# WxuanYuan/diffusynth

Measured on AMD Instinct MI355X. Metric: denoising-steps/sec (batch x T) on 256x64 latents, higher is better.
Workload: dtype bf16x3; 1 GPU; BASELINE configs[2]: DiffSynthSampler.sample() wall-clock, production ConditionedUnet (random init, torch.manual_seed(0)), bf16x3 (fp32 tensors, dense convolutions as 3 bf16 MFMA terms with fp32 accumulation: meets 1e-3 vs the fp32 reference), batch 64/GPU, latent (4,256,64), text condition, CFG=6.0 (U-Net batch 128 per step), 33-step respaced ddpm schedule, Philox noise on device; global_batch=64, parallelism=batch-shard x1, weights replicated

## Files before the change

### __graft_entry__.py

```python
import glob
import os
import subprocess
import sys

ROOT = os.path.dirname(os.path.abspath(__file__))
CSRC = os.path.join(ROOT, "diffusynth_amd", "csrc")
LIB = os.path.join(ROOT, "diffusynth_amd", "libdiffusynth_hip.so")
HIPCC = os.environ.get("HIPCC", "/opt/rocm/bin/hipcc")


NOSLP = {"conv3x3_halo3.hip", "conv3x3_halo3_hp.hip", "conv_quad_halo3.hip", "conv_quad_halo3_split.hip", "conv3x3_smalln.hip", "conv_igemm.hip", "conv_splitk.hip", "conv1x1_x3.hip", "attn_fused.hip", "attn_x3.hip", "dec_final.hip", "conv3x3_c80.hip", "convt4x4_c80.hip"}


def _compile(src, obj, flags):
    extra = ["-fno-slp-vectorize"] if (os.path.basename(src) in NOSLP and os.environ.get("DS_BUILD_SLP") != "1") else []
    cmd = [HIPCC, "--offload-arch=gfx950", "-O3", "-std=c++17", "-fPIC", "-c", "-o", obj, src] + extra + flags
    print("[build]", " ".join(cmd), flush=True)
    subprocess.check_call(cmd)


def build_lib(lib=LIB, flags=(), objdir=None, force=False):
    from concurrent.futures import ThreadPoolExecutor
    srcs = sorted(glob.glob(os.path.join(CSRC, "*.hip")))
    hdrs = glob.glob(os.path.join(CSRC, "*.hpp")) + [os.path.join(ROOT, "include", "diffusynth_hip.h")]
    objdir = objdir or os.path.join(ROOT, "build", os.path.splitext(os.path.basename(lib))[0])
    os.makedirs(objdir, exist_ok=True)
    stamp = os.path.join(objdir, "flags.txt")
    want = " ".join(sorted(flags)) + " | noslp: " + " ".join(sorted(NOSLP)) + " | slp=" + os.environ.get("DS_BUILD_SLP", "0") + " | " + HIPCC
    have = open(stamp).read() if os.path.exists(stamp) else None
    if have != want:
        force = True
        if os.path.exists(stamp):
            os.remove(stamp)
    newest_hdr = max(os.path.getmtime(h) for h in hdrs)
    jobs, objs = [], []
    for s in srcs:
        o = os.path.join(objdir, os.path.basename(s)[:-4] + ".o")
        objs.append(o)
        if force or not os.path.exists(o) or os.path.getmtime(o) < max(os.path.getmtime(s), newest_hdr):
            jobs.append((s, o))
    if jobs:
        with ThreadPoolExecutor(max_workers=min(len(jobs), os.cpu_count() or 4)) as ex:
            list(ex.map(lambda so: _compile(so[0], so[1], list(flags)), jobs))
    if jobs or not os.path.exists(lib) or os.path.getmtime(lib) < max(os.path.getmtime(o) for o in objs):
        cmd = [HIPCC, "--offload-arch=gfx950", "-fPIC", "-shared", "-o", lib] + objs
        print("[build]", " ".join(cmd), flush=True)
        subprocess.check_call(cmd)
    with open(stamp, "w") as f:
        f.write(want)
    return lib


BOUNDS_LIB = os.path.join(ROOT, "diffusynth_amd", "libdiffusynth_hip_bounds.so")


def build_bounds(force=False):
    return build_lib(BOUNDS_LIB, flags=["-DDS_BOUNDS=1"], force=force)


def build(force=False):
    build_lib(force=force)
    if os.environ.get("DS_BUILD_BOUNDS", "1") != "0":
        try:
            build_bounds(force=force)
# ... 62 lines not shown
```

### diffusynth_amd/csrc/conv3x3_halo3.hip

```cpp
#include "conv3x3_halo3_kernel.hpp"

int ds_conv3x3_halo3_hp_run(const ds_conv_params* p, dim3 grid, bool pair, hipStream_t st);

int ds_conv3x3_halo3_parts(const ds_conv_params* p) {
    const int twl = halo_twl(p->W), TW = 1 << twl, TH = BM >> twl;
    return ((p->H + TH - 1) / TH) * ((p->W + TW - 1) / TW) * (p->cout_pad / BN);
}

static int halo3_batch(const ds_conv_params* p) { return p->batch_hint > 0 ? p->batch_hint : p->B; }

int ds_conv3x3_halo3_launch(const ds_conv_params* p, hipStream_t st) {
    DS_REQUIRE(p->dtype == DS_BF16, "conv3x3_halo3: bf16 only");
    DS_REQUIRE(p->KH == 3 && p->KW == 3 && p->stride == 1 && p->pad_h == 1 && p->pad_w == 1 && !p->transposed,
               "conv3x3_halo3: 3x3 stride 1 pad 1 only");
    DS_REQUIRE(p->C1 == 0 && p->C0 % 32 == 0, "conv3x3_halo3: single source, Cin multiple of 32 (got %d+%d)", p->C0, p->C1);
    DS_REQUIRE(p->Ho == p->H && p->Wo == p->W && !p->out_nchw_f32, "conv3x3_halo3: same-size NHWC output only");
    DS_REQUIRE(p->cout_pad % BN == 0 && p->wk_order == 1, "conv3x3_halo3: cout_pad %% 96 == 0 and chunk-major weights (wk_order = 1)");
    const bool split_in = (p->flags & DS_CONV_F_SPLIT_IN) != 0;
    DS_REQUIRE(p->ksplit <= 1 || (p->slab && (p->flags == 0 || split_in) && ((split_in ? p->C0 / 64 : p->C0 / 32) % p->ksplit) == 0 && !p->res_steps),
               "conv3x3_halo3: ksplit=%d needs a slab, must divide the %d source chunks and excludes the fused res_conv", p->ksplit, split_in ? p->C0 / 64 : p->C0 / 32);
    const int out_mode = (p->flags >> 1) & 3;
    DS_REQUIRE(out_mode <= 2 && (p->flags & ~7) == 0, "conv3x3_halo3: unknown flags %d", p->flags);
    DS_REQUIRE(!split_in || (p->C0 % 64 == 0 && !p->res_steps), "conv3x3_halo3: split input needs C0 = 2C with C %% 32 == 0 and no fused res_conv");
    DS_REQUIRE(p->flags == 0 || split_in, "conv3x3_halo3: the split-precision launches (flags != 0) take a split input (DS_CONV_F_SPLIT_IN)");
    DS_REQUIRE(out_mode == 0 || !p->res_steps, "conv3x3_halo3: split / fp32 output excludes the fused res_conv");
    DS_REQUIRE(out_mode != 2 || p->act == DS_ACT_NONE, "conv3x3_halo3: fp32 output has no activation variant");
    DS_REQUIRE(!p->res || out_mode == 2 || p->flags == 0, "conv3x3_halo3: in the split-precision modes a residual needs the fp32 output");
    DS_REQUIRE(out_mode != 1 || p->out_C >= p->out_c0 + 2 * p->Cout, "conv3x3_halo3: split output needs out_C >= 2 Cout");
    const int nchunks = split_in ? (p->C0 / 32) * 3 / 2 : p->C0 / 32;
    if (p->res_steps) {
        DS_REQUIRE(!p->res, "conv3x3_halo3: a fused res_conv excludes a residual tensor");
        DS_REQUIRE(p->res_src0 && p->res_C0 > 0 && p->res_C0 % 32 == 0 && p->res_C1 % 32 == 0 && p->res_steps == (p->res_C0 + p->res_C1) / 32 &&
                       p->res_steps % 3 == 0,
                   "conv3x3_halo3: res_conv channels (%d,%d) must be multiples of 32 (96 in total) and res_steps = their chunks", p->res_C0, p->res_C1);
        DS_REQUIRE(p->res_C1 == 0 || (p->res_src1 && p->res_H1 > 0 && p->res_W1 > 0), "conv3x3_halo3: second res_conv source incomplete");
        DS_REQUIRE(ds_aligned16(p->res_src0) && (!p->res_C1 || ds_aligned16(p->res_src1)), "conv3x3_halo3: res_conv sources must be 16-byte aligned");
    }
    DS_REQUIRE((long long)p->H * p->W * (p->C0 > p->res_C0 ? p->C0 : p->res_C0) * 2 < (1ll << 31) &&
                   (long long)(nchunks * 9 + p->res_steps) * p->cout_pad * 64 < (1ll << 31),
               "conv3x3_halo3: one sample / the packed weights must stay below 2 GiB (32-bit buffer offsets)");
    DS_REQUIRE((long long)p->H * p->W * p->out_C * (out_mode == 2 ? 4 : 2) < (1ll << 31), "conv3x3_halo3: one output sample must stay below 2 GiB (32-bit buffer offsets)");
    const int twl = halo_twl(p->W), TW = 1 << twl, TH = BM >> twl;
    const bool pair = p->flags != 0 && twl == 3 && 2 * p->H <= TH && p->W <= TW && p->ksplit <= 1 && !p->res_steps && halo3_batch(p) >= 2;
    dim3 grid(((p->H + TH - 1) / TH) * ((p->W + TW - 1) / TW), p->cout_pad / BN, pair ? (p->B + 1) / 2 : p->B * (p->ksplit > 1 ? p->ksplit : 1));
    {
        static DsDevOnce once;
        int dev;
        if (once.need(&dev)) {
            float h[GELU_TAB_N];
            auto T = [](double a) { return a * 0.5 * erfc(a * 0.70710678118654752440); };
            for (int i = 0; i < GELU_TAB_N; ++i) {
                const unsigned lo = (unsigned)(GELU_TAB_BASE + i) << 16, hi = lo + 0x10000u;
                float flo, fhi;
                memcpy(&flo, &lo, 4);
                memcpy(&fhi, &hi, 4);
                h[i] = (float)T(0.5 * ((double)flo + (double)fhi));
            }
            hipError_t e = hipMemcpyToSymbol(HIP_SYMBOL(g_gelu_lut), h, sizeof(h));
            if (e != hipSuccess) DS_FAIL(DS_ELAUNCH, "conv3x3_halo3: GELU table upload: %s", hipGetErrorString(e));
            once.done(dev);
        }
    }
    return p->flags ? ds_conv3x3_halo3_hp_run(p, grid, pair, st) : halo3_run<false>(*p, grid, false, st);
}

#if DS_BOUNDS
extern "C" int ds_bounds_fetch_conv_halo3(ds_bounds_rec* out, int reset) { return ds_bounds_fetch_tu(out, reset); }
#endif
```

### diffusynth_amd/csrc/conv3x3_halo3_kernel.hpp

```cpp
#pragma once
#include "common.hpp"
#ifndef DS_STAMP
#define DS_STAMP 0
#endif
#if DS_BOUNDS
void ds_conv_bounds_table(const ds_conv_params& p, int kernel, int stats_parts, ds_bx* out);
#endif

#include "conv_halo3_common.hpp"

namespace {

__device__ __attribute__((aligned(16))) float g_gelu_lut[GELU_TAB_N];

constexpr int hp_tile(int s) { return s < 18 ? (s & 1) * 9 + (s >> 1) : s; }
constexpr int hp_tile_ahead(int s, int d) { return s + d < 27 ? hp_tile(s + d) : 27 + hp_tile(s + d - 27); }
template <int FIRST, int... I, class F>
__device__ __forceinline__ void hp_steps(std::integer_sequence<int, I...>, F&& f) { (f(std::integral_constant<int, FIRST + I>{}), ...); }

#ifdef DS_FORCE_VGPRS
#define DS_VGPR_ATTR __attribute__((amdgpu_num_vgpr(DS_FORCE_VGPRS)))
#else
#define DS_VGPR_ATTR
#endif
template <int TWL, bool HP, bool PAIR = false>
__global__ __launch_bounds__(NT, PAIR ? 1 : DS_MINBLK) DS_VGPR_ATTR void conv3x3_halo3_kernel(const ds_conv_params p) {
    static_assert(!PAIR || (HP && TWL == 3), "two samples per block: the 8 x 32 tile of the split-precision instantiation");
    using G = HG<TWL>;
    constexpr int TW = G::TW, TH = G::TH, HCP = G::HCP, NPX = G::NPX, H_IT = G::H_IT, HH0 = G::HH0, HH1 = G::HH1;
    extern __shared__ __attribute__((aligned(16))) char smem[];
    float* const shl = reinterpret_cast<float*>(smem + OFF_SHL);
    float* const red = reinterpret_cast<float*>(smem + OFF_B);

    const int tid = threadIdx.x, lane = tid & 63, wave = tid >> 6;
    const long st_k0 = DS_STAMP ? __builtin_amdgcn_s_memrealtime() : 0;
    const int m = lane & 15, q = lane >> 4;
    const int tiles_w = (p.W + TW - 1) >> TWL;
    const int gx = gridDim.x, gy = gridDim.y, nwg = gx * gy * gridDim.z;
    int wid = blockIdx.x + gx * (blockIdx.y + gy * blockIdx.z);
    if ((nwg & 7) == 0) wid = (wid & 7) * (nwg >> 3) + (wid >> 3);
    constexpr int NGROUP = 2;
    int by, bxz;
    if (gy % NGROUP == 0 && gy > NGROUP) {
        const int lo = wid % NGROUP, t = wid / NGROUP, nxz = gx * (int)gridDim.z;
        bxz = t % nxz;
        by = (t / nxz) * NGROUP + lo;
    } else {
        by = wid % gy;
        bxz = wid / gy;
    }
    const int bx = bxz % gx, bz = bxz / gx;
    const int th = bx / tiles_w, tw = bx - th * tiles_w;
    const int h0 = th * TH, w0 = tw * TW;
    const int ksplit = p.ksplit > 1 ? p.ksplit : 1;
    const int b = (PAIR ? 2 : 1) * (bz / ksplit), kz = bz - (bz / ksplit) * ksplit, n0 = by * BN;
    const bool has2 = PAIR && b + 1 < p.B;
    constexpr bool split_in = HP;
    const int Cin = p.C0, NSRC = Cin >> 5;
    const int NCC = (split_in ? NSRC + (NSRC >> 1) : NSRC) / ksplit;
    const int cc_lo = kz * NCC;
    const int nsteps = NCC * 9;
    auto src_chunk = [&](int cc) {
        const int v = cc_lo + cc;
        if (!split_in) return v;
        const int c = v / 3, j = v - 3 * c;
        return j == 2 ? (NSRC >> 1) + c : c;
    };

    const int NR = (HP || ksplit > 1) ? 0 : p.res_steps, R0 = p.res_C0 >> 5;
    const char* const wbase = reinterpret_cast<const char*>(p.wpk);
    const unsigned wbytes = (unsigned)(NCC * ksplit * 9 + p.res_steps) * p.cout_pad * 64;
    const rsrc_t rs_w = __builtin_amdgcn_make_buffer_rsrc(const_cast<char*>(wbase), (short)0, (int)wbytes, 0x00020000);

    unsigned hvo[H_IT];
    rsrc_t rs_h;
    const char* hbase;
    int h_buf = DS_BX_SRC0;
    auto use_source = [&](const void* ptr, int sH, int sW, int sC, int offh, int offw, bool centre_only, int bounds_buf) {
        hbase = reinterpret_cast<const char*>(ptr) + (size_t)b * sH * sW * sC * 2;
        rs_h = __builtin_amdgcn_make_buffer_rsrc(const_cast<char*>(hbase), (short)0, (int)((unsigned)sH * sW * sC * 2) * (has2 ? 2 : 1), 0x00020000);
// ... 47 lines not shown
    };
    auto store_b = [&](auto slotc, auto bufc) {
        constexpr int sl = decltype(slotc)::value, buf = decltype(bufc)::value;
        *reinterpret_cast<u32x4*>(smem + buf * B_STRIDE + bst0) = rb[sl][0];
        *reinterpret_cast<u32x4*>(smem + buf * B_STRIDE + bst1) = rb[sl][1];
    };
    auto load_halo_to = [&](u32x4* dst, auto halfc) {
        constexpr int half = decltype(halfc)::value, n = half ? HH1 : HH0;
#pragma unroll
        for (int k = 0; k < n; ++k) dst[k] = buf_ld16(rs_h, hbase, hvo[half * HH0 + k], h_so, h_buf);
    };
    auto load_halo = [&](auto halfc) { load_halo_to(rh, halfc); };
    auto store_halo_from = [&](const u32x4* src, auto bufc, auto halfc) {
        constexpr int buf = decltype(bufc)::value, half = decltype(halfc)::value, n = half ? HH1 : HH0;
#pragma unroll
        for (int k = 0; k < n; ++k) *reinterpret_cast<u32x4*>(smem + lds_h + buf * G::HB + (half * HH0 + k) * 64 * PSTR) = src[k];
    };
    auto store_halo = [&](auto bufc, auto halfc) { store_halo_from(rh, bufc, halfc); };

    int xb[XT];
#pragma unroll
    for (int i = 0; i < XT; ++i) {
        int row_l, col_l;
        halo_tile_rc<TWL>(wave, i, m, row_l, col_l);
        const int hp0 = (row_l + (PAIR ? 2 * (row_l >> 4) : 0)) * HCP + col_l;
        xb[i] = OFF_H + hp0 * PSTR + ((q ^ (((hp0 >> 2) & 1) << 1)) << 4);
    }
    static_assert(((HCP >> 2) & 1) == 1 && ((2 * HCP >> 2) & 1) == 0, "tap-row swizzle flips assume HCP / 4 odd");
    const int xm1 = ((m & 3) == 3) << 5, xm2 = ((m & 3) >= 2) << 5;
    const int xm1n = xm1 ^ 32, xm2n = xm2 ^ 32;
    const int bw = OFF_B + W_ROW0(m) * PSTR + ((q ^ ((-(m >> 2)) & 3)) << 4);

    bf16x8 fx[2][XT], fw[WT];
    auto read_x = [&](auto setc, auto tyc, auto txc, int imm) {
        constexpr int set = decltype(setc)::value, ty = decltype(tyc)::value, tx = decltype(txc)::value;
#pragma unroll
        for (int i = 0; i < XT; ++i) {
            int a = xb[i];
            if constexpr (HP) {
                if constexpr (tx == 1) a ^= xm1;
                if constexpr (tx == 2) a ^= xm2;
                if constexpr (ty == 1) {
                    if constexpr (tx != 0) asm volatile("" : "+v"(a));
                    a ^= 32;
                }
            } else {
                if constexpr (tx == 0 && ty == 1) a ^= 32;
                if constexpr (tx == 1) a ^= (ty == 1 ? xm1n : xm1);
                if constexpr (tx == 2) a ^= (ty == 1 ? xm2n : xm2);
            }
            fx[set][i] = *reinterpret_cast<const bf16x8*>(smem + a + (ty * HCP + tx) * PSTR + imm);
        }
    };
#ifndef DS_HALO3_ABL
#define DS_HALO3_ABL 0
#endif
    auto read_w = [&](int j, int imm) { fw[j] = *reinterpret_cast<const bf16x8*>(smem + bw + EPI_CH(j) * PSTR + imm); };
    f32x4 acc[XT][WT];
    auto mma_j = [&](auto setc, int j) {
        constexpr int set = decltype(setc)::value;
#pragma unroll
        for (int i = 0; i < XT; ++i) acc[i][j] = __builtin_amdgcn_mfma_f32_16x16x32_bf16(fw[j], fx[set][i], acc[i][j], 0, 0, 0);
    };
    using I0 = std::integral_constant<int, 0>;
    using I1 = std::integral_constant<int, 1>;
    using I2 = std::integral_constant<int, 2>;

    GnPartialLoads gnl;
    const bool raw = ksplit > 1;
    if (p.gn_part && !raw) gn_partials_issue(p.gn_part, p.gn_parts, b, gnl);
    const bool fold = !raw && CONV_FOLD(p);
    const int ncls = fold ? p.ncls : 1;
    constexpr int ST_IT = (10 * BN + NT - 1) / NT;
#if !DS_BOUNDS
    float t1v[ST_IT], t2v[ST_IT], rbv[ST_IT];
    {
        auto tab = [&](const float* ptr, int n) {
            return __builtin_amdgcn_make_buffer_rsrc(const_cast<char*>(ptr ? reinterpret_cast<const char*>(ptr) : wbase), (short)0, ptr ? n * 4 : 0, 0x00020000);
        };
        const bool use_bias = !fold && p.bias && !raw;
        const rsrc_t rs_t1 = tab(fold ? p.fold_t1 : (use_bias ? p.bias : nullptr), fold ? ncls * p.Cout : p.Cout);
        const rsrc_t rs_t2 = tab(fold ? p.fold_t2 : nullptr, ncls * p.Cout);
        const rsrc_t rs_rb = tab((NR > 0 && p.res_bias) ? p.res_bias : nullptr, p.Cout);
#pragma unroll
        for (int k = 0; k < ST_IT; ++k) {
            const int e = tid + k * NT, cls = e / BN, n = n0 + e - cls * BN;
            const unsigned bad = ((unsigned)(e >= ncls * BN) | (unsigned)(n >= p.Cout)) << 31;
            const unsigned o = (unsigned)((fold ? cls * p.Cout : 0) + n) * 4u;
            t1v[k] = __builtin_bit_cast(float, __builtin_amdgcn_raw_buffer_load_b32(rs_t1, (int)((o & 0x7fffffffu) | bad), 0, 0));
            t2v[k] = __builtin_bit_cast(float, __builtin_amdgcn_raw_buffer_load_b32(rs_t2, (int)((o & 0x7fffffffu) | bad), 0, 0));
            rbv[k] = NR > 0 ? __builtin_bit_cast(float, __builtin_amdgcn_raw_buffer_load_b32(rs_rb, (int)((((unsigned)n * 4u) & 0x7fffffffu) | bad), 0, 0)) : 0.f;
        }
    }
#endif
    const bool use_lut = !HP && G::LUT && p.act == DS_ACT_GELU && !raw;
    static_assert(GELU_TAB_N * 4 <= 2 * NT * 16 && GELU_TAB_N % 4 == 0, "the table is staged as two 16-byte vectors per thread");
    u32x4 lutv = {0u, 0u, 0u, 0u}, lutv2 = {0u, 0u, 0u, 0u};
    if (use_lut) {
        lutv = *reinterpret_cast<const u32x4*>(reinterpret_cast<const char*>(g_gelu_lut) + tid * 16);
        lutv2 = *reinterpret_cast<const u32x4*>(reinterpret_cast<const char*>(g_gelu_lut) + (NT + min(tid, GELU_TAB_N / 4 - NT - 1)) * 16);
    }
    const long st_p1 = DS_STAMP ? __builtin_amdgcn_s_memrealtime() : 0;
    u32x4 rh2[HH0];
    h_so = NR > 0 ? 0u : (unsigned)src_chunk(0) * 64u;
    load_halo_to(rh2, I0{});
    load_halo(I1{});
    if constexpr (HP) {
        load_b_at(I0{}, hp_tile(0));
        load_b_at(I1{}, hp_tile(1));
    } else {
        load_b(I0{});
        load_b(I1{});
    }
    float gn_a = 1.f, gn_am = 0.f;
    if (raw) {
    } else if (p.gn_part) gn_partials_finish(gnl, p.gn_part, p.gn_parts, p.gn_count, p.gn_eps, b, gn_a, gn_am);
    else if (p.gn_ab) {
        gn_a = DS_LD(float, p.gn_ab + 2 * b, DS_BX_GNAB);
        gn_am = DS_LD(float, p.gn_ab + 2 * b + 1, DS_BX_GNAB);
    }
    if constexpr (PAIR) {
        const int b1 = has2 ? b + 1 : b;
        float a1 = 1.f, am1 = 0.f;
        if (p.gn_part) gn_from_partials(p.gn_part, p.gn_parts, p.gn_count, p.gn_eps, b1, a1, am1);
        else if (p.gn_ab) {
            a1 = DS_LD(float, p.gn_ab + 2 * b1, DS_BX_GNAB);
            am1 = DS_LD(float, p.gn_ab + 2 * b1 + 1, DS_BX_GNAB);
        }
        if (tid == 0) {
            reinterpret_cast<float*>(smem + G::LDS)[0] = a1;
            reinterpret_cast<float*>(smem + G::LDS)[1] = am1;
        }
    }
#if DS_BOUNDS
    conv_shift_table<BN, 10, NT>(raw ? conv_kslice_view(p) : p, fold, n0, gn_am, NR > 0 ? p.res_bias : nullptr, shl);
#else
#pragma unroll
    for (int k = 0; k < ST_IT; ++k) {
        const int e = tid + k * NT;
        if (e < 10 * BN) shl[e] = (t1v[k] + rbv[k]) - gn_am * t2v[k];
    }
#endif
    const long st_p2 = DS_STAMP ? __builtin_amdgcn_s_memrealtime() : 0;
#pragma unroll
    for (int i = 0; i < XT; ++i)
#pragma unroll
        for (int j = 0; j < WT; ++j) acc[i][j] = f32x4{0.f, 0.f, 0.f, 0.f};
    if (use_lut) {
        *reinterpret_cast<u32x4*>(smem + G::OFF_LUT + tid * 16) = lutv;
        if (tid < GELU_TAB_N / 4 - NT) *reinterpret_cast<u32x4*>(smem + G::OFF_LUT + (NT + tid) * 16) = lutv2;
    }
    store_halo_from(rh2, I0{}, I0{});
    store_halo(I0{}, I1{});
    store_b(I0{}, I0{});
    store_b(I1{}, I1{});
    if constexpr (HP) {
        load_b_at(I2{}, hp_tile(2));
        load_b_at(I0{}, hp_tile(3));
        load_b_at(I1{}, hp_tile(4));
    } else {
        load_b(I2{});
        load_b(I0{});
        load_b(I1{});
    }
    __syncthreads();

    if constexpr (!HP) if (NR > 0) {
        set_res_src(1);
        load_halo_to(rh, I0{});
        load_halo_to(rh + HH0, I1{});
        auto res_step = [&](auto hbc, auto phc, int r) {
            constexpr int hb = decltype(hbc)::value, ph = decltype(phc)::value, rs = (ph + 2) % 3;
            read_x(I0{}, I1{}, I1{}, hb * G::HB);
#pragma unroll
            for (int j = 0; j < WT; ++j) read_w(j, ph * B_STRIDE);
            __builtin_amdgcn_sched_barrier(0);
            store_halo_from(rh, std::integral_constant<int, hb ^ 1>{}, I0{});
            store_halo_from(rh + HH0, std::integral_constant<int, hb ^ 1>{}, I1{});
            store_b(std::integral_constant<int, rs>{}, std::integral_constant<int, rs>{});
            __builtin_amdgcn_sched_barrier(0);
            load_b(std::integral_constant<int, rs>{});
            if (r + 2 <= NR) {
                set_res_src(r + 2);
                __builtin_amdgcn_sched_barrier(0);
                load_halo_to(rh, I0{});
                load_halo_to(rh + HH0, I1{});
            }
            __builtin_amdgcn_sched_barrier(0);
#pragma unroll
            for (int j = 0; j < WT; ++j) mma_j(I0{}, j);
            __builtin_amdgcn_sched_barrier(0);
            __syncthreads();
        };
        for (int r = 0; r < NR; r += 6) {
            res_step(I0{}, I0{}, r);
            res_step(I1{}, I1{}, r + 1);
            res_step(I0{}, I2{}, r + 2);
            if (r + 3 < NR) {
                res_step(I1{}, I0{}, r + 3);
                res_step(I0{}, I1{}, r + 4);
                res_step(I1{}, I2{}, r + 5);
            }
        }
        const float inv_a = 1.0f / gn_a;
#pragma unroll
        for (int i = 0; i < XT; ++i)
#pragma unroll
            for (int j = 0; j < WT; ++j)
#pragma unroll
                for (int r = 0; r < 4; ++r) acc[i][j][r] *= inv_a;
    }
    const int par = HP ? 0 : (NR & 1);
    if (par) read_x(I1{}, I0{}, I0{}, G::HB);
    else read_x(I0{}, I0{}, I0{}, 0);
#pragma unroll
    for (int j = 0; j < WT; ++j) read_w(j, 0);

    auto chunk = [&](auto hbufc, int cc) {
        constexpr int hbuf = decltype(hbufc)::value;
        h_so = (unsigned)src_chunk(cc + 1 < NCC ? cc + 1 : cc) * 64u;
        auto step = [&](auto tapc) {
            constexpr int tap = decltype(tapc)::value;
            constexpr int rs = (tap + 2) % 3;
            constexpr int cur = (tap + hbuf) & 1;
            constexpr int ntap = (tap + 1) % 9, nty = ntap / 3, ntx = ntap % 3, nhb = tap == 8 ? (hbuf ^ 1) : hbuf;
            constexpr int nW = 2 + (tap == 3 ? HH0 : (tap == 7 ? HH1 : 0)), nV = 2 + (tap == 1 ? HH0 : (tap == 4 ? HH1 : 0));
            if constexpr (tap == 3) store_halo(std::integral_constant<int, hbuf ^ 1>{}, I0{});
            if constexpr (tap == 7) store_halo(std::integral_constant<int, hbuf ^ 1>{}, I1{});
            store_b(std::integral_constant<int, rs>{}, std::integral_constant<int, rs>{});
            load_b(std::integral_constant<int, rs>{});
            if constexpr (tap == 1) load_halo(I0{});
            if constexpr (tap == 4) load_halo(I1{});
            mma_j(std::integral_constant<int, (DS_HALO3_ABL & 2) ? 0 : cur>{}, 0);
            if constexpr (!(DS_HALO3_ABL & 1)) read_w(0, ((tap + 1) % 3) * B_STRIDE);
            if constexpr (!(DS_HALO3_ABL & 2))
                read_x(std::integral_constant<int, cur ^ 1>{}, std::integral_constant<int, nty>{}, std::integral_constant<int, ntx>{}, nhb * G::HB);
#pragma unroll
            for (int j = 1; j < WT; ++j) {
                mma_j(std::integral_constant<int, (DS_HALO3_ABL & 2) ? 0 : cur>{}, j);
                if constexpr (!(DS_HALO3_ABL & 1)) read_w(j, ((tap + 1) % 3) * B_STRIDE);
            }
#pragma unroll
            for (int k = 0; k < nW; ++k) { SGB(SG_MFMA, 1); SGB(SG_DSW, 1); }
#pragma unroll
            for (int k = 0; k < nV; ++k) { SGB(SG_MFMA, 1); SGB(SG_VMEM, 1); }
            constexpr int L0 = nW + nV;
#pragma unroll
            for (int k = 0; k < 5; ++k) { SGB(SG_MFMA, 1); SGB(SG_DSR, 1); }
            constexpr int L1 = L0 + 5;
#pragma unroll
            for (int j = 1; j < WT; ++j) {
                const int before = (4 * j + 4 > L1 + j - 1 ? 4 * j + 4 : L1 + j - 1);
                const int prev = j == 1 ? L1 : (4 * (j - 1) + 4 > L1 + j - 2 ? 4 * (j - 1) + 4 : L1 + j - 2);
                if (before - prev == 1) SGB(SG_MFMA, 1);
                else if (before - prev == 2) SGB(SG_MFMA, 2);
                else if (before - prev == 3) SGB(SG_MFMA, 3);
                else if (before - prev == 4) SGB(SG_MFMA, 4);
                else if (before - prev == 5) SGB(SG_MFMA, 5);
                else if (before - prev == 6) SGB(SG_MFMA, 6);
                else if (before - prev == 7) SGB(SG_MFMA, 7);
                SGB(SG_DSR, 1);
            }
            __builtin_amdgcn_sched_barrier(0);
#if DS_BOUNDS || defined(DS_LGKM0)
            asm volatile("s_waitcnt lgkmcnt(0)" ::: "memory");
#else
// ... 17 lines not shown
        constexpr bool pairs = s < 18, rx = !pairs || (s & 1);
        constexpr int tap = pairs ? s >> 1 : s - 18;
        constexpr int rs = (s + 2) % 3;
        constexpr int cur = (tap + (pairs ? 0 : 1)) & 1;
        constexpr int ntap = (tap + 1) % 9, nty = ntap / 3, ntx = ntap % 3, nhb = (pairs ? 0 : 1) ^ (tap == 8 ? 1 : 0);
        constexpr int ld0 = pairs ? 2 : 19, st0 = pairs ? 6 : 21, ld1 = pairs ? 8 : 22, st1 = pairs ? 14 : 25;
        constexpr int nW = 2 + (s == st0 ? HH0 : (s == st1 ? HH1 : 0)), nV = 2 + (s == ld0 ? HH0 : (s == ld1 ? HH1 : 0));
        constexpr int NX = (rx && !(DS_HALO3_ABL & 2)) ? XT : 0;
        if constexpr (s == st0) store_halo(std::integral_constant<int, pairs ? 1 : 0>{}, I0{});
        if constexpr (s == st1) store_halo(std::integral_constant<int, pairs ? 1 : 0>{}, I1{});
        store_b(std::integral_constant<int, rs>{}, std::integral_constant<int, rs>{});
        load_b_at(std::integral_constant<int, rs>{}, hp_tile_ahead(s, 5));
        if constexpr (s == ld0) load_halo(I0{});
        if constexpr (s == ld1) load_halo(I1{});
        mma_j(std::integral_constant<int, (DS_HALO3_ABL & 2) ? 0 : cur>{}, 0);
        if constexpr (!(DS_HALO3_ABL & 1)) read_w(0, ((s + 1) % 3) * B_STRIDE);
        if constexpr (NX > 0)
            read_x(std::integral_constant<int, cur ^ 1>{}, std::integral_constant<int, nty>{}, std::integral_constant<int, ntx>{}, nhb * G::HB);
#pragma unroll
        for (int j = 1; j < WT; ++j) {
            mma_j(std::integral_constant<int, (DS_HALO3_ABL & 2) ? 0 : cur>{}, j);
            if constexpr (!(DS_HALO3_ABL & 1)) read_w(j, ((s + 1) % 3) * B_STRIDE);
        }
#pragma unroll
        for (int k = 0; k < nW; ++k) { SGB(SG_MFMA, 1); SGB(SG_DSW, 1); }
#pragma unroll
        for (int k = 0; k < nV; ++k) { SGB(SG_MFMA, 1); SGB(SG_VMEM, 1); }
#pragma unroll
        for (int k = 0; k < 1 + NX; ++k) { SGB(SG_MFMA, 1); SGB(SG_DSR, 1); }
        constexpr int L1 = nW + nV + 1 + NX;
#pragma unroll
        for (int j = 1; j < WT; ++j) {
            const int before = (4 * j + 4 > L1 + j - 1 ? 4 * j + 4 : L1 + j - 1);
            const int prev = j == 1 ? L1 : (4 * (j - 1) + 4 > L1 + j - 2 ? 4 * (j - 1) + 4 : L1 + j - 2);
            if (before - prev == 1) SGB(SG_MFMA, 1);
            else if (before - prev == 2) SGB(SG_MFMA, 2);
            else if (before - prev == 3) SGB(SG_MFMA, 3);
            else if (before - prev == 4) SGB(SG_MFMA, 4);
            else if (before - prev == 5) SGB(SG_MFMA, 5);
            else if (before - prev == 6) SGB(SG_MFMA, 6);
            else if (before - prev == 7) SGB(SG_MFMA, 7);
            SGB(SG_DSR, 1);
        }
        __builtin_amdgcn_sched_barrier(0);
#if DS_BOUNDS || defined(DS_LGKM0)
        asm volatile("s_waitcnt lgkmcnt(0)" ::: "memory");
#else
        if constexpr (rx) asm volatile("s_waitcnt lgkmcnt(10)" ::: "memory");
        else asm volatile("s_waitcnt lgkmcnt(6)" ::: "memory");
#endif
        if constexpr (!(DS_HALO3_ABL & 4)) __builtin_amdgcn_s_barrier();
        __builtin_amdgcn_sched_barrier(0);
    };
    long st_t0 = 0, st_r0 = 0;
    if constexpr (DS_STAMP) {
        st_t0 = __builtin_amdgcn_s_memtime();
        st_r0 = __builtin_amdgcn_s_memrealtime();
        __builtin_amdgcn_s_waitcnt(0xC07F);
    }
    if constexpr (HP) {
        for (int cc = 0; cc < NCC; cc += 3) {
            h_so = (unsigned)src_chunk(cc + 2) * 64u;
            hp_steps<0>(std::make_integer_sequence<int, 18>{}, hp_step);
            h_so = (unsigned)src_chunk(cc + 3 < NCC ? cc + 3 : cc) * 64u;
            hp_steps<18>(std::make_integer_sequence<int, 9>{}, hp_step);
            w_c += 27u * wstep;
        }
    } else {
        int cc0 = 0;
        if (par) {
            chunk(I1{}, 0);
            cc0 = 1;
        }
        for (int cc = cc0; cc < NCC; cc += 2) {
            chunk(I0{}, cc);
            if (cc + 1 < NCC) chunk(I1{}, cc + 1);
        }
    }

#pragma unroll
    for (int i = 0; i < XT; ++i) {
        asm volatile("" ::"v"(fx[0][i]));
        asm volatile("" ::"v"(fx[1][i]));
    }
#pragma unroll
    for (int j = 0; j < WT; ++j) asm volatile("" ::"v"(fw[j]));
    if constexpr (DS_STAMP) {
        const long st_t1 = __builtin_amdgcn_s_memtime();
        if (p.slab && lane == 0) {
            long* d = reinterpret_cast<long*>(p.slab) + ((size_t)(bz * gy + by) * gx + bx) * 32 + wave * 8;
            d[0] = st_t1 - st_t0; d[1] = st_p1 - st_k0; d[2] = st_p2 - st_k0; d[3] = nsteps;
            d[4] = st_r0 - st_k0; d[5] = __builtin_amdgcn_s_memrealtime() - st_r0; d[6] = st_k0;
        }
    }
    auto at = [&](int row_l, int col_l) {
        ConvCoord c;
        if constexpr (PAIR) {
            const int smp = row_l >> 4;
            c.ho = row_l & 15;
            c.wo = w0 + col_l;
            c.ok = c.ho < p.H && c.wo < p.W && (!smp || has2);
            c.pix = (smp * p.H + c.ho) * p.W + c.wo;
            return c;
        }
        c.ho = h0 + row_l;
        c.wo = w0 + col_l;
        c.ok = c.ho < p.H && c.wo < p.W;
        c.pix = c.ho * p.W + c.wo;
        return c;
    };
    auto coord2 = [&](int i, int mm) { int row_l, col_l; halo_tile_rc<TWL>(wave, i, mm, row_l, col_l); return at(row_l, col_l); };
    auto coord = [&](int i) { return coord2(i, m); };
    char* const stage = smem + OFF_H + wave * EPI_F32_WAVE;
    static_assert(4 * EPI_F32_WAVE <= 2 * G::HB, "the staging tiles fit the halo buffers");
    float s1 = 0.f, s2 = 0.f;
    const int outHW = p.H * p.W;
    const long st_e1 = DS_STAMP ? __builtin_amdgcn_s_memrealtime() : 0;
    const int out_mode = HP ? (p.flags >> 1) & 3 : 0;
    const float* shl_w = shl;
    float ga_w = gn_a;
    int b_e = b, outHW_e = outHW;
    if constexpr (PAIR) {
        const float gn_a1 = reinterpret_cast<const float*>(smem + G::LDS)[0], gn_am1 = reinterpret_cast<const float*>(smem + G::LDS)[1];
        float* const shl1 = reinterpret_cast<float*>(smem + OFF_H + 4 * EPI_F32_WAVE);
        static_assert(4 * EPI_F32_WAVE + SHL_BYTES <= 2 * G::HB, "the second shift table fits the halo buffers too");
        conv_shift_table<BN, 10, NT>(p, fold, n0, gn_am1, nullptr, shl1);
        __syncthreads();
        if (__builtin_amdgcn_readfirstlane(wave) >= 2) {
            shl_w = shl1;
            ga_w = gn_a1;
        }
        b_e = b >> 1;
        outHW_e = 2 * outHW;
    }
    if (raw) {
        halo3_epilogue_hp<DS_ACT_NONE, 2>(conv_kslice_view(p), acc, kz * p.B + b, n0, outHW, shl, coord, s1, s2, 1.0f, lane);
// ... 6 lines not shown
        else halo3_epilogue_rows_f32<true, false>(p, acc, b_e, n0, outHW_e, shl_w, coord, coord2, stage, s1, s2, ga_w, lane);
      } else {
        if (p.act == DS_ACT_GELU) halo3_epilogue<DS_ACT_GELU, true, false>(p, acc, b_e, n0, outHW_e, shl_w, coord, s1, s2, ga_w, lane);
        else halo3_epilogue<DS_ACT_NONE, true, false>(p, acc, b_e, n0, outHW_e, shl_w, coord, s1, s2, ga_w, lane);
      }
    } else
    if (p.act == DS_ACT_GELU) {
        const char* const lut = smem + G::OFF_LUT;
        if (use_lut) {
            if (p.res) halo3_epilogue<DS_ACT_GELU, true, true, true>(p, acc, b, n0, outHW, shl, coord, s1, s2, gn_a, lane, lut);
            else halo3_epilogue<DS_ACT_GELU, true, false, true>(p, acc, b, n0, outHW, shl, coord, s1, s2, gn_a, lane, lut);
        } else {
            if (p.res) halo3_epilogue<DS_ACT_GELU, true, true>(p, acc, b, n0, outHW, shl, coord, s1, s2, gn_a, lane);
            else halo3_epilogue<DS_ACT_GELU, true, false>(p, acc, b, n0, outHW, shl, coord, s1, s2, gn_a, lane);
        }
    } else {
        if (p.res) halo3_epilogue_rows<DS_ACT_NONE, true, true>(p, acc, b, n0, outHW, shl, coord, coord2, stage, s1, s2, gn_a, lane);
        else halo3_epilogue<DS_ACT_NONE, true, false>(p, acc, b, n0, outHW, shl, coord, s1, s2, gn_a, lane);
    }
    long st_e2 = 0, st_e3 = 0;
    if constexpr (DS_STAMP) {
        st_e2 = __builtin_amdgcn_s_memrealtime();
        __builtin_amdgcn_s_waitcnt(0x0F70);
        st_e3 = __builtin_amdgcn_s_memrealtime();
    }
    __syncthreads();
    if (p.stats_part && !raw) {
        const int parts = gridDim.x * gridDim.y;
        if constexpr (PAIR) {
            s1 = wave_sum(s1);
            s2 = wave_sum(s2);
            if (lane == 0) {
                red[2 * wave] = s1;
                red[2 * wave + 1] = s2;
            }
            __syncthreads();
            if (lane == 0 && (wave == 0 || (wave == 2 && has2))) {
                float* const dst = p.stats_part + ((size_t)(b + (wave >> 1)) * parts + by * gx + bx) * 2;
                DS_ST(float, dst, DS_BX_STATS, red[2 * wave] + red[2 * wave + 2]);
                DS_ST(float, dst + 1, DS_BX_STATS, red[2 * wave + 1] + red[2 * wave + 3]);
            }
        } else
        block_stats_write(s1, s2, red, p.stats_part + ((size_t)b * parts + by * gx + bx) * 2);
    }
    if constexpr (DS_STAMP) {
        if (p.slab && lane == 0) {
            long* d = reinterpret_cast<long*>(p.slab) + ((size_t)(bz * gy + by) * gx + bx) * 32 + wave * 8;
            d[7] = __builtin_amdgcn_s_memrealtime() - st_k0;
            if (DS_STAMP == 2) { d[1] = st_e2 - st_e1; d[2] = st_e3 - st_e2; }
        }
    }
}

template <bool HP>
int halo3_run(const ds_conv_params& p, dim3 grid, bool pair, hipStream_t st) {
    const int twl = halo_twl(p.W), out_mode = (p.flags >> 1) & 3;
    const int nchunks = HP ? (p.C0 / 32) * 3 / 2 : p.C0 / 32;
    (void)out_mode; (void)nchunks;
#if DS_BOUNDS
    {
        DsBxHost h(DS_K_CONV_HALO);
        ds_conv_bounds_table(p, DS_K_CONV_HALO, grid.x * grid.y, &h.t);
        h.set(DS_BX_W, p.wpk, (long long)(nchunks * 9 + p.res_steps) * p.cout_pad * 64);
        h.set(DS_BX_AUX0, p.res_steps ? p.res_src0 : nullptr, (long long)p.B * p.H * p.W * p.res_C0 * 2);
        h.set(DS_BX_AUX1, p.res_C1 ? p.res_src1 : nullptr, (long long)p.B * p.res_H1 * p.res_W1 * p.res_C1 * 2);
        h.set(DS_BX_AUX2, p.res_bias, (long long)p.Cout * 4);
        if (out_mode == 2) {
            if (p.ksplit <= 1) h.set(DS_BX_OUT, p.out, (long long)p.B * p.H * p.W * p.out_C * 4);
            h.set(DS_BX_RES, p.res, (long long)p.B * p.H * p.W * p.out_C * 4);
        }
        h.publish(st);
    }
#endif
    int lds = twl == 3 ? HG<3>::LDS : (twl == 4 ? HG<4>::LDS : HG<5>::LDS);
#define DS_H3_LAUNCH(TWL_, PAIR_)                                                                      \
    do {                                                                                               \
        DS_SET_MAX_LDS((conv3x3_halo3_kernel<TWL_, HP, PAIR_>), 100 * 1024, "conv3x3_halo3");          \
        hipLaunchKernelGGL((conv3x3_halo3_kernel<TWL_, HP, PAIR_>), grid, dim3(NT), lds, st, p);       \
    } while (0)
    if constexpr (HP) {
        if (pair) {
            lds += 64;
            DS_H3_LAUNCH(3, true);
        } else if (twl == 5) DS_H3_LAUNCH(5, false);
        else if (twl == 4) DS_H3_LAUNCH(4, false);
        else DS_H3_LAUNCH(3, false);
    } else {
        if (twl == 5) DS_H3_LAUNCH(5, false);
        else if (twl == 4) DS_H3_LAUNCH(4, false);
        else DS_H3_LAUNCH(3, false);
    }
#undef DS_H3_LAUNCH
    DS_CHECK_LAUNCH("conv3x3_halo3");
    return DS_OK;
}

}
```

### diffusynth_amd/csrc/misc.hip

```cpp
#include <stdarg.h>

#include "common.hpp"

static thread_local char g_err[512] = "";
void ds_set_error(const char* fmt, ...) {
    va_list ap;
    va_start(ap, fmt);
    vsnprintf(g_err, sizeof(g_err), fmt, ap);
    va_end(ap);
}
extern "C" const char* ds_last_error_string(void) { return g_err; }
extern "C" int ds_abi_version(void) { return 1; }

namespace {
__global__ __launch_bounds__(256) void split_planes_kernel(const float* x, bf16* out, size_t nvec, int CV) {
    for (size_t i = blockIdx.x * (size_t)blockDim.x + threadIdx.x; i < nvec; i += (size_t)gridDim.x * blockDim.x) {
        const size_t pix = i / CV;
        const int cv = (int)(i - pix * CV);
        const f32x4 a = *reinterpret_cast<const f32x4*>(x + i * 8), c = *reinterpret_cast<const f32x4*>(x + i * 8 + 4);
        const float v8[8] = {a[0], a[1], a[2], a[3], c[0], c[1], c[2], c[3]};
        u32x4 hi, lo;
        ds_split8(v8, hi, lo);
        bf16* o = out + (pix * 2 * CV + cv) * 8;
        *reinterpret_cast<u32x4*>(o) = hi;
        *reinterpret_cast<u32x4*>(o + (size_t)CV * 8) = lo;
    }
}
}
extern "C" int ds_split_planes(const float* x, void* out, long long npix, int C, void* stream) {
    DS_REQUIRE(x && out && npix > 0 && C > 0 && C % 8 == 0 && ds_aligned16(x) && ds_aligned16(out), "split_planes: C %% 8 == 0, 16-byte aligned pointers");
    const size_t nvec = (size_t)npix * (C / 8);
    const int blocks = (int)((nvec + 255) / 256 < 16384 ? (nvec + 255) / 256 : 16384);
    hipLaunchKernelGGL(split_planes_kernel, dim3(blocks), dim3(256), 0, reinterpret_cast<hipStream_t>(stream), x, reinterpret_cast<bf16*>(out), nvec, C / 8);
    DS_CHECK_LAUNCH("split_planes");
    return DS_OK;
}

#if DS_BOUNDS
extern "C" int ds_bounds_fetch_conv_igemm(ds_bounds_rec*, int);
extern "C" int ds_bounds_fetch_conv_splitk(ds_bounds_rec*, int);
extern "C" int ds_bounds_fetch_conv_halo3(ds_bounds_rec*, int);
extern "C" int ds_bounds_fetch_conv_halo3_hp(ds_bounds_rec*, int);
extern "C" int ds_bounds_fetch_conv_quad(ds_bounds_rec*, int);
extern "C" int ds_bounds_fetch_conv_quad_split(ds_bounds_rec*, int);
extern "C" int ds_bounds_fetch_conv_smalln(ds_bounds_rec*, int);
extern "C" int ds_bounds_fetch_dwconv_gn(ds_bounds_rec*, int);
extern "C" int ds_bounds_fetch_attn_fused(ds_bounds_rec*, int);
extern "C" int ds_bounds_fetch_attn_x3(ds_bounds_rec*, int);
extern "C" int ds_bounds_fetch_linattn(ds_bounds_rec*, int);
extern "C" int ds_bounds_fetch_conv1x1_x3(ds_bounds_rec*, int);
extern "C" int ds_bounds_fetch_conv7x7_c4(ds_bounds_rec*, int);
extern "C" int ds_bounds_fetch_convt4x4_c80(ds_bounds_rec*, int);
extern "C" int ds_bounds_fetch_conv3x3_c80(ds_bounds_rec*, int);
extern "C" int ds_bounds_fetch_conv3x3_f32_n4(ds_bounds_rec*, int);
extern "C" int ds_bounds_fetch_vq_attn(ds_bounds_rec*, int);
extern "C" int ds_bounds_fetch_ui_images(ds_bounds_rec*, int);
extern "C" int ds_bounds_fetch_arranger(ds_bounds_rec*, int);
extern "C" int ds_bounds_fetch_pitch(ds_bounds_rec*, int);
extern "C" int ds_bounds_fetch_resample_poly(ds_bounds_rec*, int);
#endif
extern "C" int ds_bounds_report(char* buf, int n, int reset) {
#if DS_BOUNDS
    static const char* knames[] = {"?", "conv_igemm", "conv3x3_halo", "splitk_reduce", "dwconv7_mfma", "dwconv7_lds", "dwconv7",
                                   "attn_fused_ctx", "attn_fused_out", "gn_apply", "linattn", "conv7x7_c4", "convt4x4_c80", "conv3x3_c80", "conv3x3_f32_n4", "vq_attn_ctx", "vq_attn_apply",
                                   "stft_images", "latent_image", "pv_stft", "pv_vocode", "pv_istft", "resample_sinc", "peak_normalize", "mix_notes", "yin_frames", "pitch_median",
                                   "resample_poly", "mix_notes_shaped"};
    static const char* bnames[] = {"src0", "src1", "weights", "out", "res", "bias", "fold_t1", "fold_t2", "gn_ab", "gn_part", "stats_part",
                                   "aux0", "aux1", "aux2", "aux3"};
    int (*fetch[])(ds_bounds_rec*, int) = {ds_bounds_fetch_conv_igemm, ds_bounds_fetch_conv_splitk, ds_bounds_fetch_conv_halo3, ds_bounds_fetch_conv_halo3_hp, ds_bounds_fetch_conv_quad, ds_bounds_fetch_conv_quad_split, ds_bounds_fetch_conv_smalln, ds_bounds_fetch_dwconv_gn,
                                           ds_bounds_fetch_attn_fused, ds_bounds_fetch_attn_x3, ds_bounds_fetch_linattn, ds_bounds_fetch_conv1x1_x3, ds_bounds_fetch_conv7x7_c4, ds_bounds_fetch_convt4x4_c80, ds_bounds_fetch_conv3x3_c80, ds_bounds_fetch_conv3x3_f32_n4, ds_bounds_fetch_vq_attn,
                                           ds_bounds_fetch_ui_images, ds_bounds_fetch_arranger, ds_bounds_fetch_pitch, ds_bounds_fetch_resample_poly};
    int hits = 0, pos = 0;
    if (buf && n > 0) buf[0] = 0;
    for (auto f : fetch) {
        ds_bounds_rec r;
        if (f(&r, reset) != 0) return -2;
        if (r.hit) {
            ++hits;
            if (buf && pos < n)
                pos += snprintf(buf + pos, n - pos, "%s: %s access of %d bytes at offset %lld outside extent %lld (block %d,%d,%d thread %d); ",
                                knames[r.kernel > 0 && r.kernel < (int)(sizeof(knames) / sizeof(knames[0])) ? r.kernel : 0], bnames[r.buf < DS_BX_N ? r.buf : 0], r.size, r.off, r.extent, r.bx, r.by,
                                r.bz, r.tid);
        }
    }
    return hits;
#else
    if (buf && n > 0) snprintf(buf, n, "not a bounds build (compile with -DDS_BOUNDS=1: tools/build_variants.py bounds)");
    (void)reset;
    return -1;
#endif
}

namespace {

__global__ void sinusoid_kernel(const int64_t* t, const float* freqs, int B, int half, float* out) {
    const int i = blockIdx.x * blockDim.x + threadIdx.x;
    if (i >= B * half) return;
    const int b = i / half, j = i % half;
    const float arg = (float)t[b] * freqs[j];
    out[(size_t)b * 2 * half + j] = sinf(arg);
    out[(size_t)b * 2 * half + half + j] = cosf(arg);
}

__global__ __launch_bounds__(256) void linear_kernel(const float* x, int xs, const float* W, const float* bias, int B, int K,
                                                     int O, int act_in, float* y, int ys) {
    const long wid = ((long)blockIdx.x * blockDim.x + threadIdx.x) >> 6;
    const int lane = threadIdx.x & 63;
    if (wid >= (long)B * O) return;
    const int b = wid / O, o = wid % O;
    const float* xr = x + (size_t)b * xs;
    const float* wr = W + (size_t)o * K;
    float acc = 0.f;
    for (int k = lane; k < K; k += 64) acc = fmaf(act_apply(xr[k], act_in), wr[k], acc);
    acc = wave_sum(acc);
    if (lane == 0) y[(size_t)b * ys + o] = acc + (bias ? bias[o] : 0.f);
}

template <int NBT>
__global__ __launch_bounds__(256) void linear_mfma_kernel(const float* x, int xs, const float* W, const float* bias, int B, int K, int O,
                                                          int act_in, float* y, int ys) {
    const int wave = (blockIdx.x * 256 + threadIdx.x) >> 6, lane = threadIdx.x & 63;
    const int o0 = wave * 16;
// ... 236 lines not shown
```

Measured before the change: 728.7 denoising-steps/s.

## Add column-walk tap order to split-precision halo3 conv for fragment reuse

Adds a COL instantiation of the split-precision 3x3 halo conv kernel. It walks the 9 taps column by column and keeps an 8-slot ring of input fragments, so that each step reloads only the new rows from LDS and reuses the rows already in registers. The aim is fewer LDS reads per MFMA in the bf16x3 conv loop. Unpaired whole-K launches now go to this path. The larger fragment ring adds register pressure, and the hand-written schedule-group barriers may not interleave well.

Result: no change. 735.4 denoising-steps/s, median of 6 (+0.9%).

```diff
diff --git a/__graft_entry__.py b/__graft_entry__.py
--- a/__graft_entry__.py
+++ b/__graft_entry__.py
@@ -9,7 +9,7 @@
 HIPCC = os.environ.get("HIPCC", "/opt/rocm/bin/hipcc")
 
 
-NOSLP = {"conv3x3_halo3.hip", "conv3x3_halo3_hp.hip", "conv_quad_halo3.hip", "conv_quad_halo3_split.hip", "conv3x3_smalln.hip", "conv_igemm.hip", "conv_splitk.hip", "conv1x1_x3.hip", "attn_fused.hip", "attn_x3.hip", "dec_final.hip", "conv3x3_c80.hip", "convt4x4_c80.hip"}
+NOSLP = {"conv3x3_halo3.hip", "conv3x3_halo3_hp.hip", "conv3x3_halo3_col.hip", "conv_quad_halo3.hip", "conv_quad_halo3_split.hip", "conv3x3_smalln.hip", "conv_igemm.hip", "conv_splitk.hip", "conv1x1_x3.hip", "attn_fused.hip", "attn_x3.hip", "dec_final.hip", "conv3x3_c80.hip", "convt4x4_c80.hip"}
 
 
 def _compile(src, obj, flags):
diff --git a/diffusynth_amd/csrc/conv3x3_halo3.hip b/diffusynth_amd/csrc/conv3x3_halo3.hip
--- a/diffusynth_amd/csrc/conv3x3_halo3.hip
+++ b/diffusynth_amd/csrc/conv3x3_halo3.hip
@@ -1,6 +1,7 @@
 #include "conv3x3_halo3_kernel.hpp"
 
 int ds_conv3x3_halo3_hp_run(const ds_conv_params* p, dim3 grid, bool pair, hipStream_t st);
+int ds_conv3x3_halo3_col_run(const ds_conv_params* p, dim3 grid, hipStream_t st);
 
 int ds_conv3x3_halo3_parts(const ds_conv_params* p) {
     const int twl = halo_twl(p->W), TW = 1 << twl, TH = BM >> twl;
@@ -61,7 +62,8 @@
             once.done(dev);
         }
     }
-    return p->flags ? ds_conv3x3_halo3_hp_run(p, grid, pair, st) : halo3_run<false>(*p, grid, false, st);
+    if (!p->flags) return halo3_run<false>(*p, grid, false, st);
+    return (p->ksplit <= 1 && !pair) ? ds_conv3x3_halo3_col_run(p, grid, st) : ds_conv3x3_halo3_hp_run(p, grid, pair, st);
 }
 
 #if DS_BOUNDS
diff --git a/diffusynth_amd/csrc/conv3x3_halo3_col.hip b/diffusynth_amd/csrc/conv3x3_halo3_col.hip
--- /dev/null
+++ b/diffusynth_amd/csrc/conv3x3_halo3_col.hip
@@ -0,0 +1,7 @@
+#include "conv3x3_halo3_kernel.hpp"
+
+int ds_conv3x3_halo3_col_run(const ds_conv_params* p, dim3 grid, hipStream_t st) { return halo3_run<true, true>(*p, grid, false, st); }
+
+#if DS_BOUNDS
+extern "C" int ds_bounds_fetch_conv_halo3_col(ds_bounds_rec* out, int reset) { return ds_bounds_fetch_tu(out, reset); }
+#endif
diff --git a/diffusynth_amd/csrc/conv3x3_halo3_kernel.hpp b/diffusynth_amd/csrc/conv3x3_halo3_kernel.hpp
--- a/diffusynth_amd/csrc/conv3x3_halo3_kernel.hpp
+++ b/diffusynth_amd/csrc/conv3x3_halo3_kernel.hpp
@@ -15,6 +15,29 @@
 
 constexpr int hp_tile(int s) { return s < 18 ? (s & 1) * 9 + (s >> 1) : s; }
 constexpr int hp_tile_ahead(int s, int d) { return s + d < 27 ? hp_tile(s + d) : 27 + hp_tile(s + d - 27); }
+constexpr int col_tap(int k) { return (k % 3) * 3 + k / 3; }
+constexpr int colhp_tile(int s) { return s < 18 ? (s & 1) * 9 + col_tap(s >> 1) : 18 + col_tap(s - 18); }
+template <bool COL> constexpr int hp_tile_of(int s) { return COL ? colhp_tile(s) : hp_tile(s); }
+template <bool COL> constexpr int hp_tile_ahead_of(int s, int d) { return s + d < 27 ? hp_tile_of<COL>(s + d) : 27 + hp_tile_of<COL>(s + d - 27); }
+template <int TWL> constexpr int col_slot(int cpar, int i, int ty) {
+    if (TWL == 5) return 2 * ((i >> 1) + ty) + (i & 1);
+    const int r = i + ty;
+    return (cpar && (r == 2 || r == 3)) ? r + 4 : r;
+}
+template <int TWL> constexpr int col_new0(int ty) { return ty == 0 ? 0 : (TWL == 5 ? 2 : 3); }
+template <int TWL> constexpr bool col_slots_ok() {
+    for (int c = 0; c < 6; ++c)
+        for (int ty = 0; ty < 3; ++ty) {
+            const int nc = ty == 2 ? (c + 1) % 6 : c, nty = (ty + 1) % 3, n0 = col_new0<TWL>(nty);
+            for (int n = n0; n < 4; ++n)
+                for (int i = 0; i < 4; ++i)
+                    if (col_slot<TWL>(nc & 1, n, nty) == col_slot<TWL>(c & 1, i, ty)) return false;
+            for (int n = 0; n < n0; ++n)
+                if (col_slot<TWL>(nc & 1, n, nty) != col_slot<TWL>(c & 1, n + 4 - n0, ty)) return false;
+        }
+    return true;
+}
+static_assert(col_slots_ok<5>() && col_slots_ok<4>() && col_slots_ok<3>(), "column walk: a prefetch would overwrite a fragment in use");
 template <int FIRST, int... I, class F>
 __device__ __forceinline__ void hp_steps(std::integer_sequence<int, I...>, F&& f) { (f(std::integral_constant<int, FIRST + I>{}), ...); }
 
@@ -23,9 +46,10 @@
 #else
 #define DS_VGPR_ATTR
 #endif
-template <int TWL, bool HP, bool PAIR = false>
+template <int TWL, bool HP, bool PAIR = false, bool COL = false>
 __global__ __launch_bounds__(NT, PAIR ? 1 : DS_MINBLK) DS_VGPR_ATTR void conv3x3_halo3_kernel(const ds_conv_params p) {
     static_assert(!PAIR || (HP && TWL == 3), "two samples per block: the 8 x 32 tile of the split-precision instantiation");
+    static_assert(!COL || (HP && !PAIR), "the column walk is a form of the split-precision loop, one sample per block");
     using G = HG<TWL>;
     constexpr int TW = G::TW, TH = G::TH, HCP = G::HCP, NPX = G::NPX, H_IT = G::H_IT, HH0 = G::HH0, HH1 = G::HH1;
     extern __shared__ __attribute__((aligned(16))) char smem[];
@@ -179,6 +203,14 @@
             fx[set][i] = *reinterpret_cast<const bf16x8*>(smem + a + (ty * HCP + tx) * PSTR + imm);
         }
     };
+    bf16x8 fc[COL ? 8 : 1];
+    auto read_xc = [&](int slot, int i, int ty, int tx, int imm) {
+        const int r = (TWL == 5 ? (i >> 1) : i) + ty;
+        int a = xb[TWL == 5 ? 2 * (r & 1) + (i & 1) : (r & 1)];
+        if (tx == 1) a ^= xm1;
+        if (tx == 2) a ^= xm2;
+        fc[slot] = *reinterpret_cast<const bf16x8*>(smem + a + ((r >> 1) * 2 * HCP + tx) * PSTR + imm);
+    };
 #ifndef DS_HALO3_ABL
 #define DS_HALO3_ABL 0
 #endif
@@ -233,8 +265,8 @@
     load_halo_to(rh2, I0{});
     load_halo(I1{});
     if constexpr (HP) {
-        load_b_at(I0{}, hp_tile(0));
-        load_b_at(I1{}, hp_tile(1));
+        load_b_at(I0{}, hp_tile_of<COL>(0));
+        load_b_at(I1{}, hp_tile_of<COL>(1));
     } else {
         load_b(I0{});
         load_b(I1{});
@@ -282,9 +314,9 @@
     store_b(I0{}, I0{});
     store_b(I1{}, I1{});
     if constexpr (HP) {
-        load_b_at(I2{}, hp_tile(2));
-        load_b_at(I0{}, hp_tile(3));
-        load_b_at(I1{}, hp_tile(4));
+        load_b_at(I2{}, hp_tile_of<COL>(2));
+        load_b_at(I0{}, hp_tile_of<COL>(3));
+        load_b_at(I1{}, hp_tile_of<COL>(4));
     } else {
         load_b(I2{});
         load_b(I0{});
@@ -338,7 +370,10 @@
                 for (int r = 0; r < 4; ++r) acc[i][j][r] *= inv_a;
     }
     const int par = HP ? 0 : (NR & 1);
-    if (par) read_x(I1{}, I0{}, I0{}, G::HB);
+    if constexpr (COL) {
+#pragma unroll
+        for (int i = 0; i < XT; ++i) read_xc(col_slot<TWL>(0, i, 0), i, 0, 0, 0);
+    } else if (par) read_x(I1{}, I0{}, I0{}, G::HB);
     else read_x(I0{}, I0{}, I0{}, 0);
 #pragma unroll
     for (int j = 0; j < WT; ++j) read_w(j, 0);
@@ -462,6 +497,66 @@
         if constexpr (!(DS_HALO3_ABL & 4)) __builtin_amdgcn_s_barrier();
         __builtin_amdgcn_sched_barrier(0);
     };
+    auto hpc_step = [&](auto stc) {
+        constexpr int s = decltype(stc)::value;
+        constexpr bool pairs = s < 18, rx = !pairs || (s & 1);
+        constexpr int k = pairs ? s >> 1 : s - 18, ty = k % 3, cpar = ((pairs ? 0 : 3) + k / 3) & 1;
+        constexpr int rs = (s + 2) % 3;
+        constexpr int nk = (k + 1) % 9, nty = nk % 3, ntx = nk / 3, nhb = (pairs ? 0 : 1) ^ (k == 8 ? 1 : 0);
+        constexpr int ncpar = k == 8 ? (pairs ? 1 : 0) : ((pairs ? 0 : 3) + ntx) & 1;
+        constexpr int ld0 = pairs ? 2 : 19, st0 = pairs ? 6 : 21, ld1 = pairs ? 8 : 22, st1 = pairs ? 14 : 25;
+        constexpr int nW = 2 + (s == st0 ? HH0 : (s == st1 ? HH1 : 0)), nV = 2 + (s == ld0 ? HH0 : (s == ld1 ? HH1 : 0));
+        constexpr int N0 = col_new0<TWL>(nty), NX = rx ? XT - N0 : 0;
+        auto mma_c = [&](int j) {
+#pragma unroll
+            for (int i = 0; i < XT; ++i) acc[i][j] = __builtin_amdgcn_mfma_f32_16x16x32_bf16(fw[j], fc[col_slot<TWL>(cpar, i, ty)], acc[i][j], 0, 0, 0);
+        };
+        if constexpr (s == st0) store_halo(std::integral_constant<int, pairs ? 1 : 0>{}, I0{});
+        if constexpr (s == st1) store_halo(std::integral_constant<int, pairs ? 1 : 0>{}, I1{});
+        store_b(std::integral_constant<int, rs>{}, std::integral_constant<int, rs>{});
+        load_b_at(std::integral_constant<int, rs>{}, hp_tile_ahead_of<true>(s, 5));
+        if constexpr (s == ld0) load_halo(I0{});
+        if constexpr (s == ld1) load_halo(I1{});
+        mma_c(0);
+        read_w(0, ((s + 1) % 3) * B_STRIDE);
+        if constexpr (NX > 0) {
+#pragma unroll
+            for (int n = N0; n < XT; ++n) read_xc(col_slot<TWL>(ncpar, n, nty), n, nty, ntx, nhb * G::HB);
+        }
+#pragma unroll
+        for (int j = 1; j < WT; ++j) {
+            mma_c(j);
+            read_w(j, ((s + 1) % 3) * B_STRIDE);
+        }
+#pragma unroll
+        for (int k2 = 0; k2 < nW; ++k2) { SGB(SG_MFMA, 1); SGB(SG_DSW, 1); }
+#pragma unroll
+        for (int k2 = 0; k2 < nV; ++k2) { SGB(SG_MFMA, 1); SGB(SG_VMEM, 1); }
+#pragma unroll
+        for (int k2 = 0; k2 < 1 + NX; ++k2) { SGB(SG_MFMA, 1); SGB(SG_DSR, 1); }
+        constexpr int L1 = nW + nV + 1 + NX;
+#pragma unroll
+        for (int j = 1; j < WT; ++j) {
+            const int before = (4 * j + 4 > L1 + j - 1 ? 4 * j + 4 : L1 + j - 1);
+            const int prev = j == 1 ? L1 : (4 * (j - 1) + 4 > L1 + j - 2 ? 4 * (j - 1) + 4 : L1 + j - 2);
+            if (before - prev == 1) SGB(SG_MFMA, 1);
+            else if (before - prev == 2) SGB(SG_MFMA, 2);
+            else if (before - prev == 3) SGB(SG_MFMA, 3);
+            else if (before - prev == 4) SGB(SG_MFMA, 4);
+            else if (before - prev == 5) SGB(SG_MFMA, 5);
+            else if (before - prev == 6) SGB(SG_MFMA, 6);
+            else if (before - prev == 7) SGB(SG_MFMA, 7);
+            SGB(SG_DSR, 1);
+        }
+        __builtin_amdgcn_sched_barrier(0);
+#if DS_BOUNDS || defined(DS_LGKM0)
+        asm volatile("s_waitcnt lgkmcnt(0)" ::: "memory");
+#else
+        asm volatile("s_waitcnt lgkmcnt(%0)" ::"n"(6 + NX) : "memory");
+#endif
+        __builtin_amdgcn_s_barrier();
+        __builtin_amdgcn_sched_barrier(0);
+    };
     long st_t0 = 0, st_r0 = 0;
     if constexpr (DS_STAMP) {
         st_t0 = __builtin_amdgcn_s_memtime();
@@ -471,9 +566,11 @@
     if constexpr (HP) {
         for (int cc = 0; cc < NCC; cc += 3) {
             h_so = (unsigned)src_chunk(cc + 2) * 64u;
-            hp_steps<0>(std::make_integer_sequence<int, 18>{}, hp_step);
+            if constexpr (COL) hp_steps<0>(std::make_integer_sequence<int, 18>{}, hpc_step);
+            else hp_steps<0>(std::make_integer_sequence<int, 18>{}, hp_step);
             h_so = (unsigned)src_chunk(cc + 3 < NCC ? cc + 3 : cc) * 64u;
-            hp_steps<18>(std::make_integer_sequence<int, 9>{}, hp_step);
+            if constexpr (COL) hp_steps<18>(std::make_integer_sequence<int, 9>{}, hpc_step);
+            else hp_steps<18>(std::make_integer_sequence<int, 9>{}, hp_step);
             w_c += 27u * wstep;
         }
     } else {
@@ -488,10 +585,15 @@
         }
     }
 
-#pragma unroll
-    for (int i = 0; i < XT; ++i) {
-        asm volatile("" ::"v"(fx[0][i]));
-        asm volatile("" ::"v"(fx[1][i]));
+    if constexpr (COL) {
+#pragma unroll
+        for (int i = 0; i < 8; ++i) asm volatile("" ::"v"(fc[i]));
+    } else {
+#pragma unroll
+        for (int i = 0; i < XT; ++i) {
+            asm volatile("" ::"v"(fx[0][i]));
+            asm volatile("" ::"v"(fx[1][i]));
+        }
     }
 #pragma unroll
     for (int j = 0; j < WT; ++j) asm volatile("" ::"v"(fw[j]));
@@ -604,7 +706,7 @@
     }
 }
 
-template <bool HP>
+template <bool HP, bool COL = false>
 int halo3_run(const ds_conv_params& p, dim3 grid, bool pair, hipStream_t st) {
     const int twl = halo_twl(p.W), out_mode = (p.flags >> 1) & 3;
     const int nchunks = HP ? (p.C0 / 32) * 3 / 2 : p.C0 / 32;
@@ -627,10 +729,15 @@
     int lds = twl == 3 ? HG<3>::LDS : (twl == 4 ? HG<4>::LDS : HG<5>::LDS);
 #define DS_H3_LAUNCH(TWL_, PAIR_)                                                                      \
     do {                                                                                               \
-        DS_SET_MAX_LDS((conv3x3_halo3_kernel<TWL_, HP, PAIR_>), 100 * 1024, "conv3x3_halo3");          \
-        hipLaunchKernelGGL((conv3x3_halo3_kernel<TWL_, HP, PAIR_>), grid, dim3(NT), lds, st, p);       \
+        DS_SET_MAX_LDS((conv3x3_halo3_kernel<TWL_, HP, PAIR_, COL>), 100 * 1024, "conv3x3_halo3");     \
+        hipLaunchKernelGGL((conv3x3_halo3_kernel<TWL_, HP, PAIR_, COL>), grid, dim3(NT), lds, st, p);  \
     } while (0)
-    if constexpr (HP) {
+    if constexpr (COL) {
+        DS_REQUIRE(!pair && p.ksplit <= 1, "conv3x3_halo3: the column-walk kernels take whole-K, unpaired launches only");
+        if (twl == 5) DS_H3_LAUNCH(5, false);
+        else if (twl == 4) DS_H3_LAUNCH(4, false);
+        else DS_H3_LAUNCH(3, false);
+    } else if constexpr (HP) {
         if (pair) {
             lds += 64;
             DS_H3_LAUNCH(3, true);
diff --git a/diffusynth_amd/csrc/misc.hip b/diffusynth_amd/csrc/misc.hip
--- a/diffusynth_amd/csrc/misc.hip
+++ b/diffusynth_amd/csrc/misc.hip
@@ -41,6 +41,7 @@
 extern "C" int ds_bounds_fetch_conv_splitk(ds_bounds_rec*, int);
 extern "C" int ds_bounds_fetch_conv_halo3(ds_bounds_rec*, int);
 extern "C" int ds_bounds_fetch_conv_halo3_hp(ds_bounds_rec*, int);
+extern "C" int ds_bounds_fetch_conv_halo3_col(ds_bounds_rec*, int);
 extern "C" int ds_bounds_fetch_conv_quad(ds_bounds_rec*, int);
 extern "C" int ds_bounds_fetch_conv_quad_split(ds_bounds_rec*, int);
 extern "C" int ds_bounds_fetch_conv_smalln(ds_bounds_rec*, int);
@@ -67,7 +68,7 @@
                                    "resample_poly", "mix_notes_shaped"};
     static const char* bnames[] = {"src0", "src1", "weights", "out", "res", "bias", "fold_t1", "fold_t2", "gn_ab", "gn_part", "stats_part",
                                    "aux0", "aux1", "aux2", "aux3"};
-    int (*fetch[])(ds_bounds_rec*, int) = {ds_bounds_fetch_conv_igemm, ds_bounds_fetch_conv_splitk, ds_bounds_fetch_conv_halo3, ds_bounds_fetch_conv_halo3_hp, ds_bounds_fetch_conv_quad, ds_bounds_fetch_conv_quad_split, ds_bounds_fetch_conv_smalln, ds_bounds_fetch_dwconv_gn,
+    int (*fetch[])(ds_bounds_rec*, int) = {ds_bounds_fetch_conv_igemm, ds_bounds_fetch_conv_splitk, ds_bounds_fetch_conv_halo3, ds_bounds_fetch_conv_halo3_hp, ds_bounds_fetch_conv_halo3_col, ds_bounds_fetch_conv_quad, ds_bounds_fetch_conv_quad_split, ds_bounds_fetch_conv_smalln, ds_bounds_fetch_dwconv_gn,
                                            ds_bounds_fetch_attn_fused, ds_bounds_fetch_attn_x3, ds_bounds_fetch_linattn, ds_bounds_fetch_conv1x1_x3, ds_bounds_fetch_conv7x7_c4, ds_bounds_fetch_convt4x4_c80, ds_bounds_fetch_conv3x3_c80, ds_bounds_fetch_conv3x3_f32_n4, ds_bounds_fetch_vq_attn,
                                            ds_bounds_fetch_ui_images, ds_bounds_fetch_arranger, ds_bounds_fetch_pitch, ds_bounds_fetch_resample_poly};
     int hits = 0, pos = 0;
```
